# ebiggers/libdeflate

Measured on AMD Instinct MI355X. Metric: compress+decompress MB/s, 64 KiB chunks level 6, higher is better.
Workload: dtype u8

## Files before the change

### libdeflate_amd/csrc/deflate_blockend.h

```cpp

static __device__ u32 block_scan(lds_t *L, u32 v, u32 *total)
{
	const u32 lane = threadIdx.x & 63, wave = threadIdx.x >> 6;
	u32 incl = wave_scan_incl(v);

	if (lane == 63)
		L->scan[0][wave] = incl;
	__syncthreads();
	const u32 sw = lane < NWAVES ? L->scan[0][lane] : 0;
	const u32 iw = wave_scan_incl(sw);
	const u32 base = bcast_lane(iw - sw, wave);
	__syncthreads();
	*total = bcast_lane(iw, NWAVES - 1);
	return base + incl - v;
}

static __device__ u32 block_scan1(lds_t *L, u32 v, u32 *total,
				  u32 *tog)
{
	const u32 lane = threadIdx.x & 63, wave = threadIdx.x >> 6;
	u32 incl = wave_scan_incl(v);
	u32 *sc = L->scan[*tog];

	*tog ^= 1;
	if (lane == 63)
		sc[wave] = incl;
	__syncthreads();
	const u32 sw = lane < NWAVES ? sc[lane] : 0;
	const u32 iw = wave_scan_incl(sw);
	*total = bcast_lane(iw, NWAVES - 1);
	return bcast_lane(iw - sw, wave) + incl - v;
}

static __device__ __forceinline__ void
length_code(u32 len, u32 *slot, u32 *xbits, u32 *xval)
{
	u32 l = len - 3;
	if (l < 8) {
		*slot = l; *xbits = 0; *xval = 0;
	} else if (len == 258) {
		*slot = 28; *xbits = 0; *xval = 0;
	} else {
		u32 hb = 31 - __builtin_clz(l);
		*xbits = hb - 2;
		*slot = 4 * (hb - 1) + ((l >> (hb - 2)) & 3);
		*xval = l & ((1u << (hb - 2)) - 1);
	}
}

static __device__ __forceinline__ void
dist_code(u32 dist, u32 *slot, u32 *xbits, u32 *xval)
{
	u32 d = dist - 1;
	if (d < 4) {
		*slot = d; *xbits = 0; *xval = 0;
	} else {
		u32 hb = 31 - __builtin_clz(d);
		*xbits = hb - 1;
		*slot = 2 * hb + ((d >> (hb - 1)) & 1);
		*xval = d & ((1u << (hb - 1)) - 1);
	}
}


struct outstate {
	u8 *out;
	u64 avail;
	u64 sg;
	u64 bits;
};

static __device__ __forceinline__ u32 *stg_of(lds_t *L)
{
	return (u32 *)L->nxtA;
}

static __device__ __forceinline__ void
stg_put(lds_t *L, const struct outstate *os, u64 bitpos, u64 code,
	u32 nbits)
{
	if (!nbits)
		return;
	u64 rel = bitpos - 8 * os->sg;
	u32 w = (u32)(rel >> 5), s = (u32)rel & 31;
	u32 *stg = stg_of(L);
	u64 lo = code << s;
	atomicOr((u32 *)&stg[w], (u32)lo);
	if (s + nbits > 32)
		atomicOr((u32 *)&stg[w + 1], (u32)(lo >> 32));
	if (s + nbits > 64)
		atomicOr((u32 *)&stg[w + 2], (u32)(code >> (64 - s)));
}

static __device__ __forceinline__ void
stg_flush(lds_t *L, struct outstate *os, bool final)
{
	u32 *stg = stg_of(L);
	u8 *stgb = (u8 *)stg;
	const u32 tid = threadIdx.x;
	u64 done_bytes = final ? (os->bits + 7) / 8 : os->bits / 8;
	u64 rel_end = done_bytes - os->sg;
	s64 first = -(s64)os->sg;
	u32 start = first > 0 ? (u32)first : 0;
	u32 units = final ? (u32)((rel_end + 15) / 16) : (u32)(rel_end / 16);

	__syncthreads();
	for (u32 u = tid; u < units; u += NT) {
		u32 b0 = u * 16, b1 = b0 + 16;
		u8 *g = os->out + (s64)(os->sg + b0);
		if (b0 >= start && b1 <= rel_end) {
			*(uint4 *)g = *(const uint4 *)(stgb + b0);
		} else {
			for (u32 b = b0 < start ? start : b0; b < b1 && b < rel_end; b++)
				g[b - b0] = stgb[b];
		}
	}
// ... 134 lines not shown
static __device__ __forceinline__ void
encode_tokens(lds_t *L, struct outstate *os, const u32 *__restrict__ tokg, u32 nseq,
	      u32 *tog, u32 tid)
{
	const u32 *tab = L->M;
	u32 *stg = stg_of(L);
	const u32 mis = ((u32)(uintptr_t)tokg >> 2) & (ENC_K - 1);
	const uint4 *__restrict__ tok4 = (const uint4 *)(tokg - mis);
	const u32 end = nseq + mis;

	uint4 nxt = make_uint4(0, 0, 0, 0);
	if (ENC_K * tid < end)
		nxt = tok4[tid];
	for (u32 b0 = 0; b0 < end; b0 += ENC_K * NT) {
		const u32 i0 = b0 + ENC_K * tid;
		const uint4 t = nxt;
		if (i0 + ENC_K * NT < end)
			nxt = tok4[(i0 + ENC_K * NT) / ENC_K];
		u32 n0, n1, n2, n3;
		const u64 v0 = enc_token(tab, t.x, i0 >= mis && i0 < end, &n0);
		const u64 v1 = enc_token(tab, t.y, i0 + 1 >= mis && i0 + 1 < end, &n1);
		const u64 v2 = enc_token(tab, t.z, i0 + 2 >= mis && i0 + 2 < end, &n2);
		const u64 v3 = enc_token(tab, t.w, i0 + 3 >= mis && i0 + 3 < end, &n3);
		const u32 nb = n0 + n1 + n2 + n3;
		u32 tot;
		const u32 off = block_scan1(L, nb, &tot, tog);
		const u32 p = (u32)(os->bits - 8 * os->sg) + off;
		const u32 w = p >> 5, s = p & 31;
		u64 a[4];
		enc_acc<0>(a, v0, s);
		enc_acc<1>(a, v1, s + n0);
		enc_acc<2>(a, v2, s + n0 + n1);
		enc_acc<3>(a, v3, s + n0 + n1 + n2);
		if (nb) {
			const u32 last = (s + nb - 1) >> 5;
			const u32 wd[7] = { (u32)a[0], (u32)(a[0] >> 32), (u32)a[1], (u32)(a[1] >> 32),
					    (u32)a[2], (u32)(a[2] >> 32), (u32)a[3] };
			atomicOr(&stg[w], wd[0]);
#pragma unroll
			for (u32 i = 1; i < 7; i++) {
				if (i < last)
					stg[w + i] = wd[i];
				else if (i == last)
					atomicOr(&stg[w + i], wd[i]);
			}
		}
		os->bits += tot;
		if (os->bits - 8 * os->sg + 48 * ENC_K * NT + 64 > 32 * STG_WORDS)
			stg_flush(L, os, false);
	}
	stg_flush(L, os, false);
}
#endif

static __device__ __forceinline__ bool
block_emit(lds_t *L, struct outstate *os, const u32 *__restrict__ tokg, u32 nseq,
	   const u8 *__restrict__ inp, u32 bstart, u32 blen, u32 is_final,
	   bool stored_only, u32 ftr_bytes, u32 *tog, u32 tid, u32 lane, u32 wave)
{
	PROF_DECL;
	PROF_START();
	u32 btype = 0;
	if (!stored_only) {
		if (tid == 0)
			L->freq[256]++;
		__syncthreads();
		{
			u32 *keys = L->M;
			u32 *usedv = L->M + 320;
			u16 *sortedO = (u16 *)(L->M + 324);
			if (tid < 2)
				usedv[tid] = 0;
			__syncthreads();
			for (u32 vt = tid; vt < 320; vt += NT) {
				const u32 f = L->freq[vt];
				if (f) {
					if (vt < 288)
						keys[atomicAdd(&usedv[0], 1u)] = (f << 9) | vt;
					else
						keys[288 + atomicAdd(&usedv[1], 1u)] =
							(f << 9) | (vt - 288);
				}
			}
			__syncthreads();
			{
				const u32 m1 = usedv[0], m2 = usedv[1];
				for (u32 i = tid; i < m1 + m2; i += NT) {
					const bool lit = i < m1;
					const u32 lo = lit ? 0 : 288, m = lit ? m1 : m2;
					const u32 key = keys[lit ? i : 288 + i - m1];
					u32 r = 0;
					for (u32 q = 0; q < m; q++)
						r += keys[lo + q] < key;
					if (lit)
						L->sorted[r] = (u16)(key & 511);
					else
						sortedO[r] = (u16)(key & 511);
				}
			}
			__syncthreads();
			PROF_MARK(10);
			if (wave == 0)
				make_code(L->freq, 288, 15, L->lens, L->codes,
					  L->sorted, HUFF_LITLEN(L),
					  usedv[0], true, lane);
			else if (wave == 1)
				make_code(L->freq + 288, 32, 15, L->lens + 288,
					  L->codes + 288, sortedO,
					  (huff_scratch<32> *)L->hw,
					  usedv[1], true, lane);
		}
		__syncthreads();
		PROF_MARK(11);
		{
			u32 *starts = L->M;
			if (tid == 0) {
// ... 90 lines not shown
						}
						atomicAdd((u32 *)&L->pre_freq[16], n16);
						atomicAdd((u32 *)&L->pre_freq[rvj], 1u);
					}
					if (left)
						atomicAdd((u32 *)&L->pre_freq[rvj], left);
					while (left) {
						L->pre_items[at++] = (u16)rvj;
						left--;
					}
				}
			}
			if (tid == 0)
				L->vars[V_NPRE] = ni;
		}
		__syncthreads();
		PROF_MARK(23);
		if (wave == 0)
			make_code(L->pre_freq, 19, 7, L->pre_lens, L->pre_codes,
				  L->sorted, (huff_scratch<32> *)L->hw,
				  0, false, lane);
		__syncthreads();
		PROF_MARK(22);
		u32 dyn = 0, stat = 0;
		for (u32 vt = tid; vt < 320; vt += NT) {
			u32 f = L->freq[vt];
			u32 xb = 0, sl = 8;
			if (vt < 288) {
				sl = vt < 144 ? 8 : vt < 256 ? 9 : vt < 280 ? 7 : 8;
				if (vt >= 265 && vt < 285)
					xb = (vt - 261) >> 2;
			} else {
				u32 ds = vt - 288;
				sl = 5;
				if (ds >= 4)
					xb = (ds >> 1) - 1;
			}
			dyn += f * (L->lens[vt] + xb);
			stat += f * (sl + xb);
		}
		if (tid < 19) {
			u32 xb = tid == 16 ? 2 : tid == 17 ? 3 : tid == 18 ? 7 : 0;
			dyn += L->pre_freq[tid] * (L->pre_lens[tid] + xb);
		}
		u32 dyn_tot, stat_tot;
		(void)block_scan(L, dyn, &dyn_tot);
		(void)block_scan(L, stat, &stat_tot);
		static const u8 perm[19] = { 16, 17, 18, 0, 8, 7, 9, 6, 10,
					     5, 11, 4, 12, 3, 13, 2, 14,
					     1, 15 };
		u32 nexp = 19;
		while (nexp > 4 && L->pre_lens[perm[nexp - 1]] == 0)
			nexp--;
		u32 cost_dyn = 3 + 5 + 5 + 4 + 3 * nexp + dyn_tot;
		u32 cost_stat = 3 + stat_tot;
		u32 pieces = blen ? (blen + 65534) / 65535 : 1;
		u32 pad = (u32)((0 - (os->bits + 3)) & 7);
		u64 cost_stored = 3 + pad + 32 + 8ull * blen +
				  (u64)(pieces - 1) * 40;
		u64 best = cost_stored;
		btype = 0;
		if (cost_stat < best) {
			best = cost_stat;
			btype = 1;
		}
		if (cost_dyn < best) {
			best = cost_dyn;
			btype = 2;
		}
		if ((os->bits + best + 7) / 8 + ftr_bytes > os->avail)
			return false;
		L->vars[V_TMP3] = nexp;
	} else {
		u32 pieces = blen ? (blen + 65534) / 65535 : 1;
		u64 cost = (u64)pieces * 40 + 8ull * blen;
		if ((os->bits + cost + 7) / 8 + ftr_bytes > os->avail)
			return false;
	}

	PROF_MARK(7);
	stg_restore(L);
	if (btype == 0) {
		u32 done = 0;
		do {
			u32 piece = blen - done > 65535 ? 65535 : blen - done;
			u32 fin = (is_final && done + piece == blen) ? 1 : 0;
			u32 pad = (u32)((0 - (os->bits + 3)) & 7);
			if (tid == 0) {
				stg_put(L, os, os->bits, fin, 3);
				u64 b = os->bits + 3 + pad;
				stg_put(L, os, b, piece | ((u64)(piece ^ 0xFFFF) << 16), 32);
			}
			os->bits += 3 + pad + 32;
			__syncthreads();
#if LDA_ENTROPY
			{
				const u8 *__restrict__ src = inp + bstart + done;
				u8 *dst = os->out + (s64)(os->bits / 8);
				u32 head = (0 - (u32)(uintptr_t)dst) & 15;
				head = head < piece ? head : piece;
				const u32 mid = (piece - head) & ~15u;
				const u32 tail = piece - head - mid;
				if (tid < head)
					stg_put(L, os, os->bits + 8 * tid, src[tid], 8);
				os->bits += 8 * head;
				stg_flush(L, os, false);
				for (u32 u = tid; u < mid / 16; u += NT) {
					uint4 v;
					__builtin_memcpy(&v, src + head + 16 * u, 16);
					*(uint4 *)(dst + head + 16 * u) = v;
				}
				if (mid) {
					os->bits += 8ull * mid;
					os->sg += mid;
				}
				__syncthreads();
				if (tid < tail)
					stg_put(L, os, os->bits + 8 * tid, src[head + mid + tid], 8);
				os->bits += 8 * tail;
				__syncthreads();
			}
#else
			for (u32 w0 = 0; w0 < piece; w0 += 2048) {
				u32 cnt = piece - w0 < 2048 ? piece - w0 : 2048;
				stg_flush(L, os, false);
				__syncthreads();
				for (u32 j = tid; j < cnt; j += NT) {
					u32 pos = bstart + done + w0 + j;
					stg_put(L, os, os->bits + 8ull * j, inp[pos], 8);
				}
				os->bits += 8ull * cnt;
				__syncthreads();
			}
// ... 83 lines not shown
#else
		__builtin_amdgcn_fence(__ATOMIC_ACQUIRE, "workgroup");
		u32 tok_nxt = tid < nseq ? tokg[tid] : 0;
		for (u32 b0 = 0; b0 < nseq; b0 += NT) {
			u64 code = 0;
			u32 nb = 0;
			const u32 tok = tok_nxt;
			if (b0 + NT + tid < nseq)
				tok_nxt = tokg[b0 + NT + tid];
			if (b0 + tid < nseq) {
				if (tok & TOK_MATCH) {
					const u32 len = (tok & 0xFF) + 3, dist = ((tok >> 8) & 0x7FFF) + 1;
					u32 sl, xb, xv, ds, dxb, dxv;
					length_code(len, &sl, &xb, &xv);
					dist_code(dist, &ds, &dxb, &dxv);
					u32 ll = L->lens[257 + sl];
					u32 dl = L->lens[288 + ds];
					u64 v = L->codes[257 + sl];
					u32 sh = ll;
					v |= (u64)xv << sh;
					sh += xb;
					v |= (u64)L->codes[288 + ds] << sh;
					sh += dl;
					v |= (u64)dxv << sh;
					sh += dxb;
					code = v;
					nb = sh;
				} else {
					code = L->codes[tok];
					nb = L->lens[tok];
				}
			}
			u32 tot;
			u32 off = block_scan1(L, nb, &tot, tog);
			stg_put(L, os, os->bits + off, code, nb);
			os->bits += tot;
			if (os->bits - 8 * os->sg + 48 * NT + 64 > 32 * STG_WORDS)
				stg_flush(L, os, false);
		}
		stg_flush(L, os, false);
#endif
		__syncthreads();
		if (tid == 0)
			stg_put(L, os, os->bits, L->codes[256], L->lens[256]);
		os->bits += L->lens[256];
		__syncthreads();
	}

	stg_save(L, os);
	PROF_MARK(8);
	return true;
}

static __device__ __forceinline__ void
finish_stream(lds_t *L, struct outstate *os, bool overflow, bool seg_last,
	      int format, u32 ftr_bytes, const u32 *__restrict__ sums, u64 c, u32 n,
	      u64 *__restrict__ out_nbytes, u32 tid)
{
	__syncthreads();
	if (!overflow && !seg_last &&
	    (os->bits + 3 + 7) / 8 + 4 > os->avail)
		overflow = true;
	if (!overflow) {
		stg_restore(L);
		if (!seg_last) {
			u64 fb = 8 * ((os->bits + 3 + 7) / 8);
			if (tid == 0)
				stg_put(L, os, fb, 0xFFFF0000ull, 32);
			os->bits = fb + 32;
			__syncthreads();
		}
		if (ftr_bytes) {
			u32 sum = sums ? sums[c] : 0;
			u64 fb = 8 * ((os->bits + 7) / 8);
			if (tid == 0) {
				if (format != LDA_FMT_ZLIB) {
					stg_put(L, os, fb, sum, 32);
					stg_put(L, os, fb + 32, n, 32);
				} else {
					stg_put(L, os, fb, __builtin_bswap32(sum), 32);
				}
			}
			os->bits = fb + 8 * ftr_bytes;
			__syncthreads();
		}
		stg_flush(L, os, true);
		const u32 size = (u32)((os->bits + 7) / 8);
		if (tid == 0)
			out_nbytes[c] = size;
		if (format == LDA_FMT_BGZF) {
			asm volatile("s_waitcnt vmcnt(0)" ::: "memory");
			__syncthreads();
			if (tid == 0) {
				const u16 bsize = (u16)(size - 1);
				__builtin_memcpy(os->out + 16, &bsize, 2);
			}
		}
	} else if (tid == 0) {
		out_nbytes[c] = 0;
	}
	__syncthreads();
}
```

### libdeflate_amd/csrc/deflate_entropy.hip

```cpp
#include <stddef.h>
#include "device_common.h"
#include "kernels.h"

#define LDA_ENTROPY 1
#define NT LDA_DEFLATE_ENTROPY_THREADS
#define VPT (1024 / NT)
#define NWAVES (NT / 64)
#ifndef ENTROPY_WGS
#define ENTROPY_WGS 4
#endif
static_assert(NT == 256, "ENTROPY_WGS waves per EU are ENTROPY_WGS workgroups per CU");
#define TOK_MATCH 0x80000000u
#define STG_WORDS 2044

struct deflate_lds {
	u32 M[1776];
	u32 freq[320];
	u8 lens[320];
	u16 codes[320];
	u16 sorted[288];
	u32 hw[288];
	u16 pre_items[320 + 8];
	u32 pre_freq[19];
	u8 pre_lens[20];
	u16 pre_codes[20];
	u32 nxtA[STG_WORDS + 8] __attribute__((aligned(16)));
	u32 scan[2][NWAVES + 1];
	u32 carry[6];
	u32 vars[4];
};
static_assert(sizeof(struct deflate_lds) * ENTROPY_WGS <= 163840, "ENTROPY_WGS workgroups per CU");

#ifdef __HIP_DEVICE_COMPILE__
#define AS3 __attribute__((address_space(3)))
#else
#define AS3
#endif
typedef AS3 struct deflate_lds lds_t;

enum { V_TMP1 = 0, V_TMP2, V_TMP3, V_NPRE, V_COUNT };
static_assert(V_COUNT <= sizeof(((struct deflate_lds *)0)->vars) / sizeof(u32), "vars[] holds them all");

#include "deflate_huffman.h"
#include "deflate_blockend.h"

extern "C" __global__ void __launch_bounds__(NT, ENTROPY_WGS)
lda_deflate_entropy_kernel(u64 n_chunks, int format, int level,
			   const u8 *__restrict__ in_base, const u64 *__restrict__ in_offsets,
			   const u64 *__restrict__ in_nbytes, u8 *__restrict__ out_base,
			   const u64 *__restrict__ out_offsets,
			   const u64 *__restrict__ out_avail_arr, u64 *__restrict__ out_nbytes,
			   const u32 *__restrict__ sums, const u32 *__restrict__ seg_info,
			   const u32 *__restrict__ tok_buf, const u32 *__restrict__ blk_buf,
			   u32 tok_stride, u32 blk_stride, u32 *__restrict__ next_chunk)
{
	extern __shared__ __attribute__((aligned(16))) u8 lds_raw[];
	lds_t *L = (lds_t *)(uintptr_t)0;
	const u32 tid = threadIdx.x, lane = tid & 63, wave = tid >> 6;
	if ((u32)(uintptr_t)(__attribute__((address_space(3))) u8 *)lds_raw != 0)
		__builtin_trap();
	if (tid == 0)
		L->vars[V_TMP1] = atomicAdd(next_chunk, 1u);
	__syncthreads();
	const u64 c = (u32)__builtin_amdgcn_readfirstlane((int)L->vars[V_TMP1]);
	if (c >= n_chunks)
		return;
	const u32 nb = blk_buf[c];
	if (nb == LDA_BLK_FUSED)
		return;
	const u32 *__restrict__ desc = blk_buf + LDA_BLK_HDR_WORDS(n_chunks) +
				       c * blk_stride * LDA_BLK_WORDS;
	const u32 *__restrict__ tokg = tok_buf + c * tok_stride;
	const u8 *__restrict__ inp = in_base + in_offsets[c];
	const u32 n = (u32)in_nbytes[c];
	const bool seg_last = seg_info ? seg_info[c] >> 31 : true;
	const u32 hdr_bytes = format == LDA_FMT_GZIP ? 10 : format == LDA_FMT_BGZF ? 18 :
			      format == LDA_FMT_ZLIB ? 2 : 0;
	const u32 ftr_bytes = format == LDA_FMT_GZIP || format == LDA_FMT_BGZF ? 8 :
			      format == LDA_FMT_ZLIB ? 4 : 0;
	bool overflow = nb == LDA_BLK_OVERFLOW;
	struct outstate os;
	os.out = out_base + out_offsets[c];
	os.avail = out_avail_arr[c];
	if (format == LDA_FMT_BGZF && os.avail > LDA_BGZF_MEMBER_MAX)
		os.avail = LDA_BGZF_MEMBER_MAX;
	os.sg = (u64)(0 - ((uintptr_t)os.out & 15));
	os.bits = 0;
	u32 tog = 0;

	for (u32 i = tid; i < STG_WORDS + 8; i += NT)
		stg_of(L)[i] = 0;
	__syncthreads();
	if (!overflow && hdr_bytes)
		put_container_header(L, &os, format, level, NULL, hdr_bytes, tid);
	__syncthreads();
	stg_save(L, &os);

	for (u32 b = 0; b < nb && !overflow; b++) {
		const u32 *__restrict__ d = desc + (size_t)b * LDA_BLK_WORDS;
		for (u32 i = tid; i < 320; i += NT)
			L->freq[i] = d[LDA_BLK_FREQ + i];
		const u32 tok0 = d[LDA_BLK_TOK0], ntok = d[LDA_BLK_NTOK];
		const u32 bstart = d[LDA_BLK_START], bend = d[LDA_BLK_END];
		const u32 flags = d[LDA_BLK_FLAGS];
		__syncthreads();
		if (!block_emit(L, &os, tokg + tok0, ntok, inp, bstart, bend - bstart, flags & 1,
				(flags & LDA_BLK_STORED) != 0, ftr_bytes, &tog, tid, lane, wave))
			overflow = true;
	}
	finish_stream(L, &os, overflow, seg_last, format, ftr_bytes, sums, c, n, out_nbytes, tid);
}

extern "C" size_t lda_deflate_entropy_lds_bytes(void)
{
	return sizeof(struct deflate_lds);
}

LDA_PROF_DEFINE_READER(libdeflate_amd_profile_read_deflate_entropy)
```

### libdeflate_amd/csrc/host_compress.hip

```cpp
#include <stdio.h>
#include <stdlib.h>
#include <string.h>
#include <atomic>
#include <new>
#include <algorithm>
#include <vector>

#include "host_objects.h"
#include "kernels.h"

using namespace lda;

struct level_cfg { uint32_t depth, nice, mode; };
static const level_cfg k_levels[13] = {
	{ 0, 0, 0 },
	{ 2, 32, 0 },
	{ 6, 10, 0 },
	{ 12, 14, 0 },
	{ 16, 30, 0 },
	{ 16, 30, 1 },
	{ 35, 65, 1 },
	{ 100, 130, 1 },
	{ 300, 258, 2 },
	{ 600, 258, 2 },
// ... 53 lines not shown
	c->pinned.release();
	c->meta.release();
	c->bgzf.release();
	c->streams.release();
	free_func_t f = c->free_func;
	c->~libdeflate_compressor();
	f(c);
}

extern "C" LIBDEFLATEAPI size_t
libdeflate_deflate_compress_bound(struct libdeflate_compressor *c, size_t n)
{
	(void)c;
	size_t blocks = (n + 4999) / 5000;
	if (blocks < 1)
		blocks = 1;
	return 5 * blocks + n;
}

extern "C" LIBDEFLATEAPI size_t
libdeflate_zlib_compress_bound(struct libdeflate_compressor *c, size_t n)
{
	return 6 + libdeflate_deflate_compress_bound(c, n);
}

extern "C" LIBDEFLATEAPI size_t
libdeflate_gzip_compress_bound(struct libdeflate_compressor *c, size_t n)
{
	return 18 + libdeflate_deflate_compress_bound(c, n);
}

static size_t dict_window(void)
{
	const size_t tile = lda_deflate_tile();
	return (32768 - 2 * tile - 272) / tile * tile;
}

struct dict_shape { uint32_t tail, pre_len, sinfo; };

static dict_shape shape_dict(int level, size_t dict_nbytes)
{
	const size_t tile = lda_deflate_tile();
	dict_shape d;
	d.tail = level == 0 ? 0 : (uint32_t)std::min(dict_nbytes, dict_window());
	d.pre_len = (uint32_t)((d.tail + tile - 1) / tile * tile);
	d.sinfo = d.pre_len | ((d.pre_len - d.tail) << 16) | 0x80000000u;
	return d;
}

#define LDA_SPLIT_SCRATCH ((size_t)1280 << 20)
#ifndef LDA_SPLIT_MIN_PER_CU
#define LDA_SPLIT_MIN_PER_CU 4
#endif

struct batch_plan {
	bool small, split;
	size_t grid, per_slice, nslices;
	uint32_t tok_stride, blk_stride;
	size_t cnt_at, sums_at, tok_at, blk_at, dict_at, total;
};

static batch_plan plan_batch(const struct libdeflate_compressor *c, size_t n,
			     size_t max_in, bool seg, bool dict)
{
	batch_plan p = {};
	p.small = max_in <= lda_deflate_small_max() && c->level <= 9 && !seg && !dict &&
		  !env_cfg().no_small;
	const size_t tile = lda_deflate_tile();
	const size_t tok_stride = align_up(max_in, 16);
	const size_t blk_stride = std::max<size_t>(1, (tok_stride + tile - 1) / tile);
	const size_t per_buf = tok_stride * 4 + blk_stride * LDA_BLK_WORDS * 4 + 4;
	const size_t num_cus = (size_t)device_ctx()->num_cus;
	p.split = !p.small && c->level <= 9 && !dict && max_in != SIZE_MAX &&
		  n >= LDA_SPLIT_MIN_PER_CU * num_cus &&
		  per_buf <= LDA_SPLIT_SCRATCH && tok_stride <= 0xFFFFFFF0u;
	p.per_slice = p.split ? std::min(n, LDA_SPLIT_SCRATCH / per_buf) : n;
	p.per_slice = std::max<size_t>(p.per_slice, 1);
	p.nslices = (n + p.per_slice - 1) / p.per_slice;
	const size_t grid_max = num_cus * (p.small ? lda_deflate_small_wgs() : 1);
	p.grid = std::min(p.per_slice, grid_max);
	p.cnt_at = p.grid * lda_deflate_seq_words() * 8;
	p.sums_at = p.cnt_at + 16 * p.nslices;
	p.dict_at = p.tok_at = align_up(p.sums_at + n * 4, 64);
	p.total = p.sums_at + n * 4;
	if (dict)
		p.total = p.dict_at + LDA_DICT_BLK_HDR + dict_window();
	if (p.split) {
		p.tok_stride = (uint32_t)tok_stride;
		p.blk_stride = (uint32_t)blk_stride;
		p.blk_at = align_up(p.tok_at + p.per_slice * tok_stride * 4, 64);
		p.total = p.blk_at + (LDA_BLK_HDR_WORDS(p.per_slice) +
				      p.per_slice * blk_stride * LDA_BLK_WORDS) * 4;
	}
	return p;
}

static int
compress_batch_impl(struct libdeflate_compressor *c, int format, size_t n,
		    const void *d_in, const uint64_t *d_in_offsets,
		    const uint64_t *d_in_nbytes, void *d_out,
		    const uint64_t *d_out_offsets, const uint64_t *d_out_avail,
		    uint64_t *d_out_nbytes, void *stream,
		    const uint32_t *d_seg_info, size_t max_in_nbytes = SIZE_MAX,
		    const void *d_dict = NULL, size_t dict_nbytes = 0)
{
	if (!c) {
		set_error("compress_batch: bad argument");
		return LIBDEFLATE_AMD_BAD_ARG;
	}
	DeviceGuard on(c->device);
	if (!on.ok())
		return LIBDEFLATE_AMD_NO_DEVICE;
	DeviceCtx *ctx = device_ctx();
	hipStream_t st = (hipStream_t)stream;

	if (!ctx)
		return LIBDEFLATE_AMD_NO_DEVICE;
	if (n == 0)
		return LIBDEFLATE_AMD_OK;
	if (!c || !d_in || !d_in_offsets || !d_in_nbytes || !d_out ||
	    !d_out_offsets || !d_out_avail || !d_out_nbytes ||
	    format < LIBDEFLATE_AMD_DEFLATE || format > LIBDEFLATE_AMD_BGZF) {
		set_error("compress_batch: bad argument");
		return LIBDEFLATE_AMD_BAD_ARG;
	}
	const bool dict = d_dict && dict_nbytes;
	const batch_plan pl = plan_batch(c, n, max_in_nbytes, d_seg_info != NULL, dict);
	const bool small = pl.small;
	uint8_t *scr = (uint8_t *)c->scratch.reserve(pl.total);
	if (!scr)
		return LIBDEFLATE_AMD_OOM;
	uint32_t *next_chunk = (uint32_t *)(scr + pl.cnt_at);
	LDA_HIP_TRY(hipMemsetAsync(next_chunk, 0, 16 * pl.nslices, st),
		    LIBDEFLATE_AMD_NO_DEVICE);
	uint8_t *blk = NULL;
	if (dict) {
		const dict_shape sh = shape_dict(c->level, dict_nbytes);
		blk = scr + pl.dict_at;
		hipLaunchKernelGGL(lda_dict_prep_kernel, dim3(1), dim3(256), 0, st,
				   (const uint8_t *)d_dict, (uint64_t)dict_nbytes, sh.tail,
				   sh.pre_len, sh.sinfo, blk);
		LDA_HIP_TRY(hipGetLastError(), LIBDEFLATE_AMD_NO_DEVICE);
		if (format == LIBDEFLATE_AMD_ZLIB) {
			int rc = libdeflate_amd_adler32_batch(1, d_dict, (const uint64_t *)(blk + 16),
							      (const uint64_t *)(blk + 24), NULL,
							      (uint32_t *)(blk + 4), stream);
			if (rc != LIBDEFLATE_AMD_OK)
				return rc;
		}
	}
	uint32_t *sums = NULL;
	if (format != LIBDEFLATE_AMD_DEFLATE) {
		sums = (uint32_t *)(scr + pl.sums_at);
		int rc = format == LIBDEFLATE_AMD_GZIP || format == LIBDEFLATE_AMD_BGZF ?
			libdeflate_amd_crc32_batch(n, d_in, d_in_offsets,
						   d_in_nbytes, NULL, sums, stream) :
			libdeflate_amd_adler32_batch(n, d_in, d_in_offsets,
						     d_in_nbytes, NULL, sums, stream);
		if (rc != LIBDEFLATE_AMD_OK)
			return rc;
	}
	const size_t lds = small ? lda_deflate_small_lds_bytes() : lda_deflate_lds_bytes();
	if (!ctx->deflate_attr_set.load(std::memory_order_acquire)) {
		LDA_HIP_TRY(hipFuncSetAttribute(
				(const void *)lda_deflate_small_kernel,
				hipFuncAttributeMaxDynamicSharedMemorySize,
				(int)lda_deflate_small_lds_bytes()), LIBDEFLATE_AMD_NO_DEVICE);
		LDA_HIP_TRY(hipFuncSetAttribute(
				(const void *)lda_deflate_batch_kernel,
				hipFuncAttributeMaxDynamicSharedMemorySize,
				(int)lda_deflate_lds_bytes()), LIBDEFLATE_AMD_NO_DEVICE);
		LDA_HIP_TRY(hipFuncSetAttribute(
				(const void *)lda_deflate_opt_kernel,
				hipFuncAttributeMaxDynamicSharedMemorySize,
				(int)lda_deflate_lds_bytes()), LIBDEFLATE_AMD_NO_DEVICE);
		LDA_HIP_TRY(hipFuncSetAttribute(
				(const void *)lda_deflate_fused_kernel,
				hipFuncAttributeMaxDynamicSharedMemorySize,
				(int)lda_deflate_lds_bytes()), LIBDEFLATE_AMD_NO_DEVICE);
		ctx->deflate_attr_set.store(true, std::memory_order_release);
	}
	const level_cfg &lv = k_levels[c->level];
	if (!pl.split && (small || lv.mode == 3)) {
		hipLaunchKernelGGL(small ? lda_deflate_small_kernel : lda_deflate_opt_kernel,
				   dim3((unsigned)pl.grid),
				   dim3(small ? LDA_DEFLATE_SMALL_THREADS : LDA_DEFLATE_THREADS),
				   lds, st, (uint64_t)n, format, c->level,
				   lv.depth, lv.nice, lv.mode, (const uint8_t *)d_in,
				   d_in_offsets, d_in_nbytes, (uint8_t *)d_out,
				   d_out_offsets, d_out_avail, d_out_nbytes, sums,
				   (uint64_t *)scr, d_seg_info, next_chunk, (const uint8_t *)blk);
		LDA_HIP_TRY(hipGetLastError(), LIBDEFLATE_AMD_NO_DEVICE);
		return LIBDEFLATE_AMD_OK;
	}
	if (!pl.split) {
		hipLaunchKernelGGL(lda_deflate_fused_kernel, dim3((unsigned)pl.grid),
				   dim3(LDA_DEFLATE_THREADS), lds, st, (uint64_t)n, format,
				   c->level, lv.depth, lv.nice, lv.mode, (const uint8_t *)d_in,
				   d_in_offsets, d_in_nbytes, (uint8_t *)d_out,
				   d_out_offsets, d_out_avail, d_out_nbytes, sums,
				   (uint64_t *)scr, d_seg_info, next_chunk, (const uint8_t *)blk,
				   (const uint32_t *)NULL, (const uint32_t *)NULL);
		LDA_HIP_TRY(hipGetLastError(), LIBDEFLATE_AMD_NO_DEVICE);
		return LIBDEFLATE_AMD_OK;
	}
	uint32_t *tok = (uint32_t *)(scr + pl.tok_at), *bd = (uint32_t *)(scr + pl.blk_at);
	for (size_t k = 0; k < pl.nslices; k++) {
		const size_t lo = k * pl.per_slice, nk = std::min(pl.per_slice, n - lo);
		const uint32_t *sk = sums ? sums + lo : NULL;
		const uint32_t *gk = d_seg_info ? d_seg_info + lo : NULL;
		hipLaunchKernelGGL(lda_deflate_batch_kernel, dim3((unsigned)std::min(nk, pl.grid)),
				   dim3(LDA_DEFLATE_THREADS), lds, st, (uint64_t)nk, format,
				   c->level, lv.depth, lv.nice, lv.mode, (const uint8_t *)d_in,
				   d_in_offsets + lo, d_in_nbytes + lo, (uint8_t *)d_out,
				   d_out_offsets + lo, d_out_avail + lo, d_out_nbytes + lo, sk,
				   (uint64_t *)scr, gk, next_chunk + k, (const uint8_t *)NULL,
				   tok, bd, pl.tok_stride, pl.blk_stride, next_chunk + 2 * pl.nslices + k);
		LDA_HIP_TRY(hipGetLastError(), LIBDEFLATE_AMD_NO_DEVICE);
		hipLaunchKernelGGL(lda_deflate_entropy_kernel, dim3((unsigned)nk),
				   dim3(LDA_DEFLATE_ENTROPY_THREADS), lda_deflate_entropy_lds_bytes(),
				   st, (uint64_t)nk, format, c->level, (const uint8_t *)d_in,
				   d_in_offsets + lo, d_in_nbytes + lo, (uint8_t *)d_out,
				   d_out_offsets + lo, d_out_avail + lo, d_out_nbytes + lo, sk, gk,
				   (const uint32_t *)tok, (const uint32_t *)bd, pl.tok_stride,
				   pl.blk_stride, next_chunk + 3 * pl.nslices + k);
		LDA_HIP_TRY(hipGetLastError(), LIBDEFLATE_AMD_NO_DEVICE);
		hipLaunchKernelGGL(lda_deflate_fused_kernel, dim3((unsigned)std::min(nk, pl.grid)),
				   dim3(LDA_DEFLATE_THREADS), lds, st, (uint64_t)nk, format,
				   c->level, lv.depth, lv.nice, lv.mode, (const uint8_t *)d_in,
				   d_in_offsets + lo, d_in_nbytes + lo, (uint8_t *)d_out,
				   d_out_offsets + lo, d_out_avail + lo, d_out_nbytes + lo, sk,
				   (uint64_t *)scr, gk, next_chunk + pl.nslices + k,
				   (const uint8_t *)NULL, (const uint32_t *)bd,
				   (const uint32_t *)(next_chunk + 2 * pl.nslices + k));
		LDA_HIP_TRY(hipGetLastError(), LIBDEFLATE_AMD_NO_DEVICE);
	}
	return LIBDEFLATE_AMD_OK;
}

extern "C" LIBDEFLATEAPI int
libdeflate_amd_compress_batch_dict(struct libdeflate_compressor *c, int format,
				   size_t n, const void *d_dict, size_t dict_nbytes,
				   const void *d_in, const uint64_t *d_in_offsets,
				   const uint64_t *d_in_nbytes, void *d_out,
				   const uint64_t *d_out_offsets,
				   const uint64_t *d_out_avail,
				   uint64_t *d_out_nbytes, void *stream)
{
	if (format != LIBDEFLATE_AMD_DEFLATE && format != LIBDEFLATE_AMD_ZLIB) {
		set_error("compress_batch_dict: format %d takes no dictionary", format);
		return LIBDEFLATE_AMD_BAD_ARG;
	}
	if (dict_nbytes && !d_dict) {
		set_error("compress_batch_dict: bad argument");
		return LIBDEFLATE_AMD_BAD_ARG;
	}
	return compress_batch_impl(c, format, n, d_in, d_in_offsets, d_in_nbytes,
				   d_out, d_out_offsets, d_out_avail,
				   d_out_nbytes, stream, NULL, SIZE_MAX, d_dict, dict_nbytes);
}

extern "C" LIBDEFLATEAPI int
libdeflate_amd_compress_batch(struct libdeflate_compressor *c, int format,
			      size_t n, const void *d_in,
			      const uint64_t *d_in_offsets,
			      const uint64_t *d_in_nbytes, void *d_out,
			      const uint64_t *d_out_offsets,
			      const uint64_t *d_out_avail,
			      uint64_t *d_out_nbytes, void *stream)
{
	return compress_batch_impl(c, format, n, d_in, d_in_offsets, d_in_nbytes,
				   d_out, d_out_offsets, d_out_avail,
				   d_out_nbytes, stream, NULL);
}

extern "C" LIBDEFLATEAPI int
libdeflate_amd_compress_batch_bounded(struct libdeflate_compressor *c, int format,
				      size_t n, const void *d_in,
// ... 447 lines not shown
```

### libdeflate_amd/csrc/kernels.h

```cpp
#ifndef LDA_KERNELS_H
#define LDA_KERNELS_H

#include <hip/hip_runtime.h>
#include <stdint.h>

extern "C" __global__ void
lda_crc32_batch_kernel(uint64_t n_chunks, const uint8_t *base,
		       const uint64_t *offsets, const uint64_t *nbytes,
		       const uint32_t *init, uint32_t *out,
		       const uint32_t *g_tables, const uint32_t *xpow8);
extern "C" __global__ void
lda_adler32_batch_kernel(uint64_t n_chunks, const uint8_t *base,
			 const uint64_t *offsets, const uint64_t *nbytes,
			 const uint32_t *init, uint32_t *out);
#define LDA_DICT_BLK_HDR 64
extern "C" __global__ void
lda_dict_prep_kernel(const uint8_t *dict, uint64_t dict_nbytes, uint32_t tail,
		     uint32_t pre_len, uint32_t sinfo, uint8_t *blk);

extern "C" __global__ void
lda_inflate_batch_kernel(uint64_t n_chunks, int format, uint32_t lpw,
			 const uint8_t *in_base,
			 const uint64_t *in_offsets, const uint64_t *in_nbytes,
			 uint8_t *out_base, const uint64_t *out_offsets,
			 const uint64_t *out_avail, int32_t *results,
			 uint64_t *actual_in, uint64_t *actual_out,
			 const uint8_t *dict, uint32_t dict_len,
			 const uint32_t *dict_id);
extern "C" __global__ void
lda_inflate_wave_kernel(uint64_t n_chunks, int format, uint32_t *tokscratch,
			uint32_t *next_stream, const uint32_t *order,
			const uint8_t *in_base,
			const uint64_t *in_offsets, const uint64_t *in_nbytes,
			uint8_t *out_base, const uint64_t *out_offsets,
			const uint64_t *out_avail, int32_t *results,
			uint64_t *actual_in, uint64_t *actual_out,
			const uint8_t *dict, uint32_t dict_len,
			const uint32_t *dict_id);
extern "C" __global__ void
lda_inflate_order_kernel(uint64_t n, const uint64_t *in_nbytes, const uint64_t *out_avail,
			 uint32_t *order);
extern "C" size_t lda_inflate_tokcap(void);
extern "C" size_t lda_inflate_window_bytes(void);
extern "C" __global__ void
lda_inflate_finalize_kernel(uint64_t n_chunks, int format, int exact_fill,
			    const uint8_t *in_base, const uint64_t *in_offsets,
			    const uint64_t *out_avail, const uint32_t *sums,
			    int32_t *results, uint64_t *actual_in,
			    uint64_t *actual_out);

#define LDA_DEFLATE_THREADS 1024
#define LDA_BLK_TOK0 0
#define LDA_BLK_NTOK 1
#define LDA_BLK_START 2
#define LDA_BLK_END 3
#define LDA_BLK_FLAGS 4
#define LDA_BLK_STORED 2u
#define LDA_BLK_FREQ 8
#define LDA_BLK_WORDS (LDA_BLK_FREQ + 320)
#define LDA_BLK_OVERFLOW 0xFFFFFFFFu
#define LDA_BLK_FUSED 0xFFFFFFFEu
#define LDA_BLK_LIST(n) (((n) + 15) / 16 * 16)
#define LDA_BLK_HDR_WORDS(n) (2 * LDA_BLK_LIST(n))
extern "C" __global__ void
lda_deflate_batch_kernel(uint64_t n_chunks, int format, int level,
			 uint32_t depth, uint32_t nice, uint32_t mode,
			 const uint8_t *in_base, const uint64_t *in_offsets,
			 const uint64_t *in_nbytes, uint8_t *out_base,
			 const uint64_t *out_offsets, const uint64_t *out_avail,
			 uint64_t *out_nbytes, const uint32_t *sums,
			 uint64_t *seq_scratch, const uint32_t *seg_info,
			 uint32_t *next_chunk, const uint8_t *dict_pre,
			 uint32_t *tok_buf, uint32_t *blk_buf, uint32_t tok_stride,
			 uint32_t blk_stride, uint32_t *fused_cnt);
extern "C" __global__ void
lda_deflate_fused_kernel(uint64_t n_chunks, int format, int level,
			 uint32_t depth, uint32_t nice, uint32_t mode,
			 const uint8_t *in_base, const uint64_t *in_offsets,
			 const uint64_t *in_nbytes, uint8_t *out_base,
			 const uint64_t *out_offsets, const uint64_t *out_avail,
			 uint64_t *out_nbytes, const uint32_t *sums,
			 uint64_t *seq_scratch, const uint32_t *seg_info,
			 uint32_t *next_chunk, const uint8_t *dict_pre,
			 const uint32_t *blk_buf, const uint32_t *fused_cnt);
#define LDA_DEFLATE_ENTROPY_THREADS 256
extern "C" __global__ void
lda_deflate_entropy_kernel(uint64_t n_chunks, int format, int level,
			   const uint8_t *in_base, const uint64_t *in_offsets,
			   const uint64_t *in_nbytes, uint8_t *out_base,
			   const uint64_t *out_offsets, const uint64_t *out_avail,
			   uint64_t *out_nbytes, const uint32_t *sums,
			   const uint32_t *seg_info, const uint32_t *tok_buf,
			   const uint32_t *blk_buf, uint32_t tok_stride,
			   uint32_t blk_stride, uint32_t *next_chunk);
extern "C" size_t lda_deflate_entropy_lds_bytes(void);
extern "C" __global__ void
lda_deflate_opt_kernel(uint64_t n_chunks, int format, int level,
		       uint32_t depth, uint32_t nice, uint32_t mode,
		       const uint8_t *in_base, const uint64_t *in_offsets,
		       const uint64_t *in_nbytes, uint8_t *out_base,
		       const uint64_t *out_offsets, const uint64_t *out_avail,
		       uint64_t *out_nbytes, const uint32_t *sums,
		       uint64_t *seq_scratch, const uint32_t *seg_info,
		       uint32_t *next_chunk, const uint8_t *dict_pre);
#define LDA_DEFLATE_SMALL_THREADS 256
extern "C" __global__ void
lda_deflate_small_kernel(uint64_t n_chunks, int format, int level,
			 uint32_t depth, uint32_t nice, uint32_t mode,
			 const uint8_t *in_base, const uint64_t *in_offsets,
			 const uint64_t *in_nbytes, uint8_t *out_base,
			 const uint64_t *out_offsets, const uint64_t *out_avail,
			 uint64_t *out_nbytes, const uint32_t *sums,
			 uint64_t *seq_scratch, const uint32_t *seg_info,
			 uint32_t *next_chunk, const uint8_t *dict_pre);
extern "C" size_t lda_deflate_small_lds_bytes(void);
extern "C" size_t lda_deflate_small_max(void);
extern "C" size_t lda_deflate_small_wgs(void);
extern "C" size_t lda_deflate_tile(void);
extern "C" size_t lda_deflate_lds_bytes(void);
extern "C" size_t lda_deflate_seq_words(void);

extern "C" size_t lda_inflate_lds_per_stream(void);
extern "C" size_t lda_inflate_lds_shared(void);

#define LDA_SCAN_BLOCK 2048
extern "C" __global__ void
lda_scan_local_kernel(uint64_t n, const uint64_t *sizes, uint64_t *offsets,
		      uint64_t *block_sums);
extern "C" __global__ void
lda_scan_blocks_kernel(uint64_t nblocks, uint64_t *block_sums);
extern "C" __global__ void
lda_compact_copy_kernel(uint64_t n, const uint8_t *in_base,
			const uint64_t *in_offsets, const uint64_t *sizes,
			uint8_t *out_base, uint64_t *offsets,
			const uint64_t *block_sums);
extern "C" __global__ void
lda_bgzf_desc_kernel(uint64_t m, uint64_t n, uint64_t *in_off, uint64_t *in_n,
		     uint64_t *slot_off, uint64_t *slot_avail);
extern "C" __global__ void
lda_bgzf_copy_kernel(uint64_t m, const uint8_t *slots, const uint64_t *sizes,
		     const uint64_t *offsets, const uint64_t *block_sums, uint8_t *out,
		     uint64_t out_avail, uint32_t eof_bytes, uint64_t *index);
extern "C" __global__ void
lda_bgzf_finalize_kernel(uint64_t m, uint64_t n, const uint64_t *sizes,
			 const uint64_t *total_at, uint8_t *out, uint64_t out_avail,
			 uint32_t eof_bytes, uint64_t *out_nbytes, uint64_t *index);

#define LDA_BR_TILE 4096
// ... 64 lines not shown
```

Measured before the change: 34580.

## Split Huffman code construction into a separate small-workgroup codes kernel

Huffman tree building and cost estimation move out of the entropy kernel into a new 128-thread kernel. That kernel writes a per-block record (lengths, codes, precode items, costs) to global scratch, and the entropy kernel loads this record into LDS before emitting bits. Without the tree scratch the entropy kernel's LDS footprint shrinks, so ENTROPY_WGS is raised from 4 to 7 workgroups per CU. The cost is an extra kernel launch per slice, plus a global write and read of roughly 1.7 KB per block.

```diff
diff --git a/libdeflate_amd/csrc/deflate_blockend.h b/libdeflate_amd/csrc/deflate_blockend.h
--- a/libdeflate_amd/csrc/deflate_blockend.h
+++ b/libdeflate_amd/csrc/deflate_blockend.h
@@ -62,6 +62,7 @@
 	}
 }
 
+#ifndef LDA_CODES
 
 struct outstate {
 	u8 *out;
@@ -302,16 +303,16 @@
 	stg_flush(L, os, false);
 }
 #endif
-
-static __device__ __forceinline__ bool
-block_emit(lds_t *L, struct outstate *os, const u32 *__restrict__ tokg, u32 nseq,
-	   const u8 *__restrict__ inp, u32 bstart, u32 blen, u32 is_final,
-	   bool stored_only, u32 ftr_bytes, u32 *tog, u32 tid, u32 lane, u32 wave)
+#endif
+
+#if !LDA_ENTROPY
+static __device__ __forceinline__ void
+block_codes(lds_t *L, u32 *dyn_tot_out, u32 *stat_tot_out, u32 *nexp_out,
+	    u32 tid, u32 lane, u32 wave)
 {
 	PROF_DECL;
 	PROF_START();
-	u32 btype = 0;
-	if (!stored_only) {
+	{
 		if (tid == 0)
 			L->freq[256]++;
 		__syncthreads();
@@ -508,6 +509,25 @@
 		u32 nexp = 19;
 		while (nexp > 4 && L->pre_lens[perm[nexp - 1]] == 0)
 			nexp--;
+		*dyn_tot_out = dyn_tot;
+		*stat_tot_out = stat_tot;
+		*nexp_out = nexp;
+	}
+	PROF_MARK(7);
+}
+#endif
+
+#ifndef LDA_CODES
+static __device__ __forceinline__ bool
+block_write(lds_t *L, struct outstate *os, const u32 *__restrict__ tokg, u32 nseq,
+	    const u8 *__restrict__ inp, u32 bstart, u32 blen, u32 is_final,
+	    bool stored_only, u32 ftr_bytes, u32 *tog, u32 tid,
+	    u32 dyn_tot, u32 stat_tot, u32 nexp)
+{
+	PROF_DECL;
+	PROF_START();
+	u32 btype = 0;
+	if (!stored_only) {
 		u32 cost_dyn = 3 + 5 + 5 + 4 + 3 * nexp + dyn_tot;
 		u32 cost_stat = 3 + stat_tot;
 		u32 pieces = blen ? (blen + 65534) / 65535 : 1;
@@ -534,7 +554,6 @@
 			return false;
 	}
 
-	PROF_MARK(7);
 	stg_restore(L);
 	if (btype == 0) {
 		u32 done = 0;
@@ -724,6 +743,21 @@
 	return true;
 }
 
+#if !LDA_ENTROPY
+static __device__ __forceinline__ bool
+block_emit(lds_t *L, struct outstate *os, const u32 *__restrict__ tokg, u32 nseq,
+	   const u8 *__restrict__ inp, u32 bstart, u32 blen, u32 is_final,
+	   bool stored_only, u32 ftr_bytes, u32 *tog, u32 tid, u32 lane, u32 wave)
+{
+	u32 dyn_tot = 0, stat_tot = 0, nexp = 0;
+
+	if (!stored_only)
+		block_codes(L, &dyn_tot, &stat_tot, &nexp, tid, lane, wave);
+	return block_write(L, os, tokg, nseq, inp, bstart, blen, is_final, stored_only,
+			   ftr_bytes, tog, tid, dyn_tot, stat_tot, nexp);
+}
+#endif
+
 static __device__ __forceinline__ void
 finish_stream(lds_t *L, struct outstate *os, bool overflow, bool seg_last,
 	      int format, u32 ftr_bytes, const u32 *__restrict__ sums, u64 c, u32 n,
@@ -773,3 +807,4 @@
 	}
 	__syncthreads();
 }
+#endif
diff --git a/libdeflate_amd/csrc/deflate_codes.hip b/libdeflate_amd/csrc/deflate_codes.hip
--- /dev/null
+++ b/libdeflate_amd/csrc/deflate_codes.hip
@@ -0,0 +1,112 @@
+#include <stddef.h>
+#include "device_common.h"
+#include "kernels.h"
+
+#define LDA_CODES 1
+#define NT LDA_DEFLATE_CODES_THREADS
+#define VPT 3
+#define NWAVES (NT / 64)
+#ifndef CODES_WAVES
+#define CODES_WAVES 8
+#endif
+static_assert(NT == 128 && NT * VPT >= 320, "two waves: one per tree; every code length has a thread");
+
+struct deflate_lds {
+	union {
+		u32 M[1776];
+		struct {
+			u32 hw[288];
+			u32 gap_[56];
+			u16 sorted[288];
+		};
+	};
+	u32 freq[320];
+	u32 pre_freq[19];
+	u32 scan[2][NWAVES + 1];
+	u8 lens[320];
+	u16 codes[320];
+	u16 pre_items[320 + 8];
+	u8 pre_lens[20];
+	u16 pre_codes[20];
+	u32 vars[4];
+	u32 cost[2];
+};
+static_assert(sizeof(struct deflate_lds) * (CODES_WAVES * 4 / NWAVES) <= 163840,
+	      "CODES_WAVES waves per SIMD are CODES_WAVES * 2 workgroups per CU");
+#define LDA_REC_AT(m) ((offsetof(struct deflate_lds, m) - offsetof(struct deflate_lds, lens)) / 4)
+static_assert(LDA_REC_AT(codes) == LDA_REC_CODES && LDA_REC_AT(pre_items) == LDA_REC_PRE_ITEMS &&
+	      LDA_REC_AT(pre_lens) == LDA_REC_PRE_LENS && LDA_REC_AT(pre_codes) == LDA_REC_PRE_CODES &&
+	      LDA_REC_AT(vars) == LDA_REC_VARS && LDA_REC_AT(cost) == LDA_REC_COST &&
+	      offsetof(struct deflate_lds, lens) % 4 == 0 &&
+	      sizeof(struct deflate_lds) - offsetof(struct deflate_lds, lens) == 4 * LDA_REC_USED,
+	      "the record is the tail of the LDS block, word for word");
+
+#ifdef __HIP_DEVICE_COMPILE__
+#define AS3 __attribute__((address_space(3)))
+#else
+#define AS3
+#endif
+typedef AS3 struct deflate_lds lds_t;
+
+enum { V_TMP1 = 0, V_TMP2, V_TMP3, V_NPRE, V_COUNT };
+static_assert(V_COUNT <= sizeof(((struct deflate_lds *)0)->vars) / sizeof(u32), "vars[] holds them all");
+
+#include "deflate_huffman.h"
+static_assert(sizeof(huff_scratch<32>) <= 320 * 4 &&
+	      offsetof(struct deflate_lds, sorted) >= 340 * 4 &&
+	      offsetof(struct deflate_lds, sorted) + sizeof(((struct deflate_lds *)0)->sorted) <= 512 * 4,
+	      "hw[] lies in the keys, sorted[] between the rank sort's words and the litlen tree's scratch");
+#include "deflate_blockend.h"
+
+extern "C" __global__ void __launch_bounds__(NT, CODES_WAVES)
+lda_deflate_codes_kernel(u64 n_chunks, const u32 *__restrict__ blk_buf, u32 blk_stride,
+			 u32 *__restrict__ rec_buf, u32 *__restrict__ next_chunk)
+{
+	extern __shared__ __attribute__((aligned(16))) u8 lds_raw[];
+	lds_t *L = (lds_t *)(uintptr_t)0;
+	const u32 tid = threadIdx.x;
+	if ((u32)(uintptr_t)(__attribute__((address_space(3))) u8 *)lds_raw != 0)
+		__builtin_trap();
+	if (tid == 0)
+		L->vars[V_TMP1] = atomicAdd(next_chunk, 1u);
+	__syncthreads();
+	const u64 c = (u32)__builtin_amdgcn_readfirstlane((int)L->vars[V_TMP1]);
+	if (c >= n_chunks)
+		return;
+	const u32 nb = blk_buf[c];
+	if (nb == LDA_BLK_FUSED || nb == LDA_BLK_OVERFLOW)
+		return;
+	const u32 *__restrict__ desc = blk_buf + LDA_BLK_HDR_WORDS(n_chunks) +
+				       c * blk_stride * LDA_BLK_WORDS;
+	u32 *__restrict__ rec = rec_buf + c * blk_stride * LDA_REC_WORDS;
+	u32 *recl = (u32 *)L->lens;
+
+	for (u32 b = 0; b < nb && b < blk_stride; b++) {
+		const u32 *__restrict__ d = desc + (size_t)b * LDA_BLK_WORDS;
+		if (d[LDA_BLK_FLAGS] & LDA_BLK_STORED)
+			continue;
+		__syncthreads();
+		for (u32 i = tid; i < 320; i += NT)
+			L->freq[i] = d[LDA_BLK_FREQ + i];
+		__syncthreads();
+		u32 dyn_tot, stat_tot, nexp;
+		u32 t = tid;
+		asm volatile("" : "+v"(t));
+		block_codes(L, &dyn_tot, &stat_tot, &nexp, t, t & 63, t >> 6);
+		if (tid == 0) {
+			L->vars[V_TMP3] = nexp;
+			L->cost[0] = dyn_tot;
+			L->cost[1] = stat_tot;
+		}
+		__syncthreads();
+		for (u32 i = tid; i < LDA_REC_USED; i += NT)
+			rec[(size_t)b * LDA_REC_WORDS + i] = recl[i];
+	}
+}
+
+extern "C" size_t lda_deflate_codes_lds_bytes(void)
+{
+	return sizeof(struct deflate_lds);
+}
+
+LDA_PROF_DEFINE_READER(libdeflate_amd_profile_read_deflate_codes)
diff --git a/libdeflate_amd/csrc/deflate_entropy.hip b/libdeflate_amd/csrc/deflate_entropy.hip
--- a/libdeflate_amd/csrc/deflate_entropy.hip
+++ b/libdeflate_amd/csrc/deflate_entropy.hip
@@ -7,29 +7,33 @@
 #define VPT (1024 / NT)
 #define NWAVES (NT / 64)
 #ifndef ENTROPY_WGS
-#define ENTROPY_WGS 4
+#define ENTROPY_WGS 7
 #endif
 static_assert(NT == 256, "ENTROPY_WGS waves per EU are ENTROPY_WGS workgroups per CU");
 #define TOK_MATCH 0x80000000u
 #define STG_WORDS 2044
 
 struct deflate_lds {
-	u32 M[1776];
-	u32 freq[320];
+	u32 nxtA[STG_WORDS + 8] __attribute__((aligned(16)));
+	u32 M[544];
+	u32 scan[2][NWAVES + 1];
+	u32 carry[6];
 	u8 lens[320];
 	u16 codes[320];
-	u16 sorted[288];
-	u32 hw[288];
 	u16 pre_items[320 + 8];
-	u32 pre_freq[19];
 	u8 pre_lens[20];
 	u16 pre_codes[20];
-	u32 nxtA[STG_WORDS + 8] __attribute__((aligned(16)));
-	u32 scan[2][NWAVES + 1];
-	u32 carry[6];
 	u32 vars[4];
+	u32 cost[2];
 };
 static_assert(sizeof(struct deflate_lds) * ENTROPY_WGS <= 163840, "ENTROPY_WGS workgroups per CU");
+#define LDA_REC_AT(m) ((offsetof(struct deflate_lds, m) - offsetof(struct deflate_lds, lens)) / 4)
+static_assert(LDA_REC_AT(codes) == LDA_REC_CODES && LDA_REC_AT(pre_items) == LDA_REC_PRE_ITEMS &&
+	      LDA_REC_AT(pre_lens) == LDA_REC_PRE_LENS && LDA_REC_AT(pre_codes) == LDA_REC_PRE_CODES &&
+	      LDA_REC_AT(vars) == LDA_REC_VARS && LDA_REC_AT(cost) == LDA_REC_COST &&
+	      offsetof(struct deflate_lds, lens) % 4 == 0 &&
+	      offsetof(struct deflate_lds, cost) + 8 - offsetof(struct deflate_lds, lens) == 4 * LDA_REC_USED,
+	      "a record is loaded as it lies, word for word");
 
 #ifdef __HIP_DEVICE_COMPILE__
 #define AS3 __attribute__((address_space(3)))
@@ -41,7 +45,6 @@
 enum { V_TMP1 = 0, V_TMP2, V_TMP3, V_NPRE, V_COUNT };
 static_assert(V_COUNT <= sizeof(((struct deflate_lds *)0)->vars) / sizeof(u32), "vars[] holds them all");
 
-#include "deflate_huffman.h"
 #include "deflate_blockend.h"
 
 extern "C" __global__ void __launch_bounds__(NT, ENTROPY_WGS)
@@ -52,11 +55,12 @@
 			   const u64 *__restrict__ out_avail_arr, u64 *__restrict__ out_nbytes,
 			   const u32 *__restrict__ sums, const u32 *__restrict__ seg_info,
 			   const u32 *__restrict__ tok_buf, const u32 *__restrict__ blk_buf,
-			   u32 tok_stride, u32 blk_stride, u32 *__restrict__ next_chunk)
+			   u32 tok_stride, u32 blk_stride, u32 *__restrict__ next_chunk,
+			   const u32 *__restrict__ rec_buf)
 {
 	extern __shared__ __attribute__((aligned(16))) u8 lds_raw[];
 	lds_t *L = (lds_t *)(uintptr_t)0;
-	const u32 tid = threadIdx.x, lane = tid & 63, wave = tid >> 6;
+	const u32 tid = threadIdx.x;
 	if ((u32)(uintptr_t)(__attribute__((address_space(3))) u8 *)lds_raw != 0)
 		__builtin_trap();
 	if (tid == 0)
@@ -70,6 +74,8 @@
 		return;
 	const u32 *__restrict__ desc = blk_buf + LDA_BLK_HDR_WORDS(n_chunks) +
 				       c * blk_stride * LDA_BLK_WORDS;
+	const u32 *__restrict__ rec = rec_buf + c * blk_stride * LDA_REC_WORDS;
+	u32 *recl = (u32 *)L->lens;
 	const u32 *__restrict__ tokg = tok_buf + c * tok_stride;
 	const u8 *__restrict__ inp = in_base + in_offsets[c];
 	const u32 n = (u32)in_nbytes[c];
@@ -98,14 +104,23 @@
 
 	for (u32 b = 0; b < nb && !overflow; b++) {
 		const u32 *__restrict__ d = desc + (size_t)b * LDA_BLK_WORDS;
-		for (u32 i = tid; i < 320; i += NT)
-			L->freq[i] = d[LDA_BLK_FREQ + i];
 		const u32 tok0 = d[LDA_BLK_TOK0], ntok = d[LDA_BLK_NTOK];
 		const u32 bstart = d[LDA_BLK_START], bend = d[LDA_BLK_END];
 		const u32 flags = d[LDA_BLK_FLAGS];
-		__syncthreads();
-		if (!block_emit(L, &os, tokg + tok0, ntok, inp, bstart, bend - bstart, flags & 1,
-				(flags & LDA_BLK_STORED) != 0, ftr_bytes, &tog, tid, lane, wave))
+		const bool stored_only = (flags & LDA_BLK_STORED) != 0;
+		u32 dyn_tot = 0, stat_tot = 0, nexp = 0;
+		if (!stored_only) {
+			for (u32 i = tid; i < LDA_REC_USED; i += NT)
+				recl[i] = rec[(size_t)b * LDA_REC_WORDS + i];
+			__syncthreads();
+			nexp = L->vars[V_TMP3];
+			dyn_tot = L->cost[0];
+			stat_tot = L->cost[1];
+		}
+		u32 t = tid;
+		asm volatile("" : "+v"(t));
+		if (!block_write(L, &os, tokg + tok0, ntok, inp, bstart, bend - bstart, flags & 1,
+				 stored_only, ftr_bytes, &tog, t, dyn_tot, stat_tot, nexp))
 			overflow = true;
 	}
 	finish_stream(L, &os, overflow, seg_last, format, ftr_bytes, sums, c, n, out_nbytes, tid);
diff --git a/libdeflate_amd/csrc/host_compress.hip b/libdeflate_amd/csrc/host_compress.hip
--- a/libdeflate_amd/csrc/host_compress.hip
+++ b/libdeflate_amd/csrc/host_compress.hip
@@ -129,12 +129,13 @@
 #ifndef LDA_SPLIT_MIN_PER_CU
 #define LDA_SPLIT_MIN_PER_CU 4
 #endif
+#define LDA_SLICE_COUNTERS 5
 
 struct batch_plan {
 	bool small, split;
 	size_t grid, per_slice, nslices;
 	uint32_t tok_stride, blk_stride;
-	size_t cnt_at, sums_at, tok_at, blk_at, dict_at, total;
+	size_t cnt_at, sums_at, tok_at, blk_at, rec_at, dict_at, total;
 };
 
 static batch_plan plan_batch(const struct libdeflate_compressor *c, size_t n,
@@ -146,7 +147,7 @@
 	const size_t tile = lda_deflate_tile();
 	const size_t tok_stride = align_up(max_in, 16);
 	const size_t blk_stride = std::max<size_t>(1, (tok_stride + tile - 1) / tile);
-	const size_t per_buf = tok_stride * 4 + blk_stride * LDA_BLK_WORDS * 4 + 4;
+	const size_t per_buf = tok_stride * 4 + blk_stride * (LDA_BLK_WORDS + LDA_REC_WORDS) * 4 + 4;
 	const size_t num_cus = (size_t)device_ctx()->num_cus;
 	p.split = !p.small && c->level <= 9 && !dict && max_in != SIZE_MAX &&
 		  n >= LDA_SPLIT_MIN_PER_CU * num_cus &&
@@ -157,7 +158,7 @@
 	const size_t grid_max = num_cus * (p.small ? lda_deflate_small_wgs() : 1);
 	p.grid = std::min(p.per_slice, grid_max);
 	p.cnt_at = p.grid * lda_deflate_seq_words() * 8;
-	p.sums_at = p.cnt_at + 16 * p.nslices;
+	p.sums_at = p.cnt_at + 4 * LDA_SLICE_COUNTERS * p.nslices;
 	p.dict_at = p.tok_at = align_up(p.sums_at + n * 4, 64);
 	p.total = p.sums_at + n * 4;
 	if (dict)
@@ -166,8 +167,9 @@
 		p.tok_stride = (uint32_t)tok_stride;
 		p.blk_stride = (uint32_t)blk_stride;
 		p.blk_at = align_up(p.tok_at + p.per_slice * tok_stride * 4, 64);
-		p.total = p.blk_at + (LDA_BLK_HDR_WORDS(p.per_slice) +
-				      p.per_slice * blk_stride * LDA_BLK_WORDS) * 4;
+		p.rec_at = align_up(p.blk_at + (LDA_BLK_HDR_WORDS(p.per_slice) +
+						p.per_slice * blk_stride * LDA_BLK_WORDS) * 4, 64);
+		p.total = p.rec_at + p.per_slice * blk_stride * LDA_REC_WORDS * 4;
 	}
 	return p;
 }
@@ -208,7 +210,7 @@
 	if (!scr)
 		return LIBDEFLATE_AMD_OOM;
 	uint32_t *next_chunk = (uint32_t *)(scr + pl.cnt_at);
-	LDA_HIP_TRY(hipMemsetAsync(next_chunk, 0, 16 * pl.nslices, st),
+	LDA_HIP_TRY(hipMemsetAsync(next_chunk, 0, 4 * LDA_SLICE_COUNTERS * pl.nslices, st),
 		    LIBDEFLATE_AMD_NO_DEVICE);
 	uint8_t *blk = NULL;
 	if (dict) {
@@ -282,6 +284,7 @@
 		return LIBDEFLATE_AMD_OK;
 	}
 	uint32_t *tok = (uint32_t *)(scr + pl.tok_at), *bd = (uint32_t *)(scr + pl.blk_at);
+	uint32_t *rec = (uint32_t *)(scr + pl.rec_at);
 	for (size_t k = 0; k < pl.nslices; k++) {
 		const size_t lo = k * pl.per_slice, nk = std::min(pl.per_slice, n - lo);
 		const uint32_t *sk = sums ? sums + lo : NULL;
@@ -294,13 +297,19 @@
 				   (uint64_t *)scr, gk, next_chunk + k, (const uint8_t *)NULL,
 				   tok, bd, pl.tok_stride, pl.blk_stride, next_chunk + 2 * pl.nslices + k);
 		LDA_HIP_TRY(hipGetLastError(), LIBDEFLATE_AMD_NO_DEVICE);
+		hipLaunchKernelGGL(lda_deflate_codes_kernel, dim3((unsigned)nk),
+				   dim3(LDA_DEFLATE_CODES_THREADS), lda_deflate_codes_lds_bytes(), st,
+				   (uint64_t)nk, (const uint32_t *)bd, pl.blk_stride, rec,
+				   next_chunk + 4 * pl.nslices + k);
+		LDA_HIP_TRY(hipGetLastError(), LIBDEFLATE_AMD_NO_DEVICE);
 		hipLaunchKernelGGL(lda_deflate_entropy_kernel, dim3((unsigned)nk),
 				   dim3(LDA_DEFLATE_ENTROPY_THREADS), lda_deflate_entropy_lds_bytes(),
 				   st, (uint64_t)nk, format, c->level, (const uint8_t *)d_in,
 				   d_in_offsets + lo, d_in_nbytes + lo, (uint8_t *)d_out,
 				   d_out_offsets + lo, d_out_avail + lo, d_out_nbytes + lo, sk, gk,
 				   (const uint32_t *)tok, (const uint32_t *)bd, pl.tok_stride,
-				   pl.blk_stride, next_chunk + 3 * pl.nslices + k);
+				   pl.blk_stride, next_chunk + 3 * pl.nslices + k,
+				   (const uint32_t *)rec);
 		LDA_HIP_TRY(hipGetLastError(), LIBDEFLATE_AMD_NO_DEVICE);
 		hipLaunchKernelGGL(lda_deflate_fused_kernel, dim3((unsigned)std::min(nk, pl.grid)),
 				   dim3(LDA_DEFLATE_THREADS), lds, st, (uint64_t)nk, format,
diff --git a/libdeflate_amd/csrc/kernels.h b/libdeflate_amd/csrc/kernels.h
--- a/libdeflate_amd/csrc/kernels.h
+++ b/libdeflate_amd/csrc/kernels.h
@@ -62,6 +62,15 @@
 #define LDA_BLK_FUSED 0xFFFFFFFEu
 #define LDA_BLK_LIST(n) (((n) + 15) / 16 * 16)
 #define LDA_BLK_HDR_WORDS(n) (2 * LDA_BLK_LIST(n))
+#define LDA_REC_LENS 0
+#define LDA_REC_CODES 80
+#define LDA_REC_PRE_ITEMS 240
+#define LDA_REC_PRE_LENS 404
+#define LDA_REC_PRE_CODES 409
+#define LDA_REC_VARS 419
+#define LDA_REC_COST 423
+#define LDA_REC_USED 425
+#define LDA_REC_WORDS 432
 extern "C" __global__ void
 lda_deflate_batch_kernel(uint64_t n_chunks, int format, int level,
 			 uint32_t depth, uint32_t nice, uint32_t mode,
@@ -92,8 +101,14 @@
 			   uint64_t *out_nbytes, const uint32_t *sums,
 			   const uint32_t *seg_info, const uint32_t *tok_buf,
 			   const uint32_t *blk_buf, uint32_t tok_stride,
-			   uint32_t blk_stride, uint32_t *next_chunk);
+			   uint32_t blk_stride, uint32_t *next_chunk,
+			   const uint32_t *rec_buf);
 extern "C" size_t lda_deflate_entropy_lds_bytes(void);
+#define LDA_DEFLATE_CODES_THREADS 128
+extern "C" __global__ void
+lda_deflate_codes_kernel(uint64_t n_chunks, const uint32_t *blk_buf, uint32_t blk_stride,
+			 uint32_t *rec_buf, uint32_t *next_chunk);
+extern "C" size_t lda_deflate_codes_lds_bytes(void);
 extern "C" __global__ void
 lda_deflate_opt_kernel(uint64_t n_chunks, int format, int level,
 		       uint32_t depth, uint32_t nice, uint32_t mode,
```

After: 34880 (median of 6 runs). No clear change (+0.9%).
